# NVIDIA/flowtron

Measured on AMD Instinct MI355X. Metric: mel-frames/sec training (2-flow, 80-mel), higher is better.
Workload: dtype bf16; 1 GPU; BASELINE configs[1]: 2-flow LJS config.json model, per-GPU batch 32, T_max=862, L_max=157, attn-prior + CTC on, fwd+loss+bwd+clip+RAdam; global_batch=32, parallelism=dp1, mfma_operands=bf16, storage=fp32, skipped_steps=0

## Files before the change

### flowtron_amd/_lib.py

```python
from __future__ import annotations

import ctypes as C
import os

import torch

_HERE = os.path.dirname(os.path.abspath(__file__))
LIB_PATH = os.path.join(_HERE, "libflowtron_hip.so")

FT_F32, FT_BF16, FT_F16 = 0, 1, 2
GEMM_SPLITK = 1
GEMM_SPLITK_DET = 2
GEMM_C16 = 4
ACT_NONE, ACT_TANH, ACT_RELU, ACT_SIGMOID = 0, 1, 2, 3

_p, _i, _l, _f, _sz, _d = C.c_void_p, C.c_int, C.c_int64, C.c_float, C.c_size_t, C.c_double


class GemmArgs(C.Structure):
    _fields_ = [("A", _p), ("B", _p), ("C", _p), ("bias", _p),
                ("M", _i), ("N", _i), ("K", _i), ("batch", _i),
                ("sAm", _l), ("sAk", _l), ("sBk", _l), ("sBn", _l), ("ldc", _l),
                ("bsA", _l), ("bsB", _l), ("bsC", _l),
                ("alpha", _f), ("beta", _f), ("act", _i), ("mode", _i), ("flags", _i),
                ("work", _p), ("work_bytes", _sz)]


class GemmImgArgs(C.Structure):
    _fields_ = [("A", _p), ("B", _p), ("C", _p), ("bias", _p), ("M", _i), ("N", _i), ("K", _i),
                ("lda", _l), ("ldb", _l), ("ldc", _l), ("a_kmajor", _i), ("b_kmajor", _i),
                ("alpha", _f), ("beta", _f), ("act", _i), ("flags", _i),
                ("rowmap", _p), ("rows_dev", _p), ("compact", _i), ("k_shift", _i), ("r1_row", _p), ("r1_col", _p),
                ("split_work", _p), ("split_work_bytes", _sz)]


class LstmFwdRole(C.Structure):
    _fields_ = [("gx", _p), ("lens", _p), ("y", _p), ("ldy", _l), ("gates", _p), ("cell", _p), ("wimg", _p), ("state_h", _p), ("state_c", _p),
                ("B", C.c_int32), ("ldb", C.c_int32), ("t0", C.c_int32), ("t1", C.c_int32), ("gx16", C.c_int32)]


class LstmBwdRole(C.Structure):
    _fields_ = [("dy", _p), ("ldy", _l), ("lens", _p), ("gates", _p), ("cell", _p), ("dgx", _p), ("wimg", _p),
                ("dimg", _p), ("dimg_ld", _l), ("dimg_rows", _l), ("dbias", _p), ("state_da", _p), ("state_dc", _p),
                ("B", C.c_int32), ("ldb", C.c_int32), ("t0", C.c_int32), ("t1", C.c_int32), ("carry_in", C.c_int32)]


class ImgDesc(C.Structure):
    _fields_ = [("src", _p), ("ld", _l), ("rows", _l), ("cols", _l), ("dst", _p), ("kind", _i)]


class CummAttnArgs(C.Structure):
    _fields_ = [(n, _p) for n in ("text", "Q", "V", "w_key", "v", "w1", "b1", "w2", "b2", "in_lens", "ctx", "attn", "logprob",
                                  "cumm_all", "kproj_all", "work")] + [("work_bytes", _sz)] + [
        (n, _i) for n in ("T", "B", "L", "E", "A", "NF", "K1", "K2")] + [("temperature", _f), ("mode", _i), ("persist_status", _p)]


# ... 212 lines not shown
```

### flowtron_amd/csrc/gemm_bf16.hip

```cpp
#include "common.h"
#include <stdlib.h>

namespace {

constexpr int TB = 128;

inline size_t up(size_t v, size_t m) { return (v + m - 1) / m * m; }

__device__ __forceinline__ uint4 pack8(const float (&v)[8]) {
    uint4 o;
    o.x = pack_op16x2(v[0], v[1]); o.y = pack_op16x2(v[2], v[3]);
    o.z = pack_op16x2(v[4], v[5]); o.w = pack_op16x2(v[6], v[7]);
    return o;
}

__device__ __forceinline__ int mapped_rows(const int* rdev, int Rp, int& Rz) {
    const int R = *rdev;
    const int z = (R + 32 + 255) & ~255;
    Rz = z < Rp ? z : Rp;
    return R;
}

__device__ __forceinline__ void img_rows_body(const float* __restrict__ src, long sr, long sc, int R, int Cc,
                                              unsigned short* __restrict__ dst, int Rp, int Cp, int vec,
// ... 173 lines not shown
}

void make_image(const float* src, long sr, long sc, int R, int Cc, unsigned short* dst, int Rp, int Cp, hipStream_t st,
                const int* rowmap = nullptr, const int* rdev = nullptr, long dld = 0) {
    const bool vec = sc == 1 && reinterpret_cast<uintptr_t>(src) % 16 == 0 && sr % 4 == 0;
    const size_t chunks = (size_t)Rp * (Cp >> 3);
    const int blocks = (int)((chunks + 255) / 256 < 16384 ? (chunks + 255) / 256 : 16384);
    hipLaunchKernelGGL(img_rows_k, dim3(blocks), dim3(256), 0, st, src, sr, sc, R, Cc, dst, Rp, Cp, vec ? 1 : 0, rowmap, rdev,
                       dld ? dld : (long)Cp);
}

struct BfP {
    const unsigned short* A; const unsigned short* B; float* C; const float* bias;
    int M, N, nk;
    long lda, ldb, ldc;
    float alpha, beta;
    int act, gx, gy, splits, ksteps;
    int vec_c;
    const int* rowmap; const int* rows_dev; int compact, k_shift;
    int chunk_w;
    const float* r1row; const float* r1col;
    long c_slice;
    int c16;
};

typedef __attribute__((address_space(3))) void lds_void;
typedef const __attribute__((address_space(1))) void glb_void;
typedef __attribute__((ext_vector_type(4))) short bf16x4;

template <bool KM, int RT = 128>
struct Operand {
    static constexpr int NS = RT / 64;
    static constexpr int WT = RT / 32;
    const unsigned short* src[NS];
    size_t kstride;
    int dst[NS];
    int roff;
    __device__ __forceinline__ void init(const unsigned short* img, long ld, int r0, int wave, int lane, int wsel) {
        const int li = lane & 15, kg = lane >> 4;
        if constexpr (!KM) {
            const int srow = lane >> 2, skp = (lane & 3) ^ ((lane >> 4) & 2);
#pragma unroll
            for (int g = 0; g < NS; ++g) {
                src[g] = img + (size_t)(r0 + (wave * NS + g) * 16 + srow) * ld + skp * 8;
                dst[g] = (wave * NS + g) << 10;
            }
// ... 69 lines not shown
        for (int g = 0; g < NS; ++g)
            __builtin_amdgcn_global_load_lds((glb_void*)(src0 + (size_t)t * 64 + (size_t)g * ld8 + ((g & 1) ? xodd : 0)),
                                             (lds_void*)(sbuf + dst0 + g * 1024), 16, 0, 0);
    }
    __device__ __forceinline__ bf16x8 frag(const unsigned char* sbuf, int i, int ks) const {
        return *reinterpret_cast<const bf16x8*>(sbuf + ((roff + (i << 11)) ^ (ks << 6)));
    }
};

template <bool AKM, bool BKM, bool SPLIT, int RTA, int KS = 32, bool SB = false>
__global__ __launch_bounds__(256, SB ? 4 : (RTA == 256 || KS == 64) ? 2 : 4) void gemm_bf16_k(BfP p) {
    static_assert(!SB || (KS == 64 && RTA == 128 && !SPLIT), "single-buffer form: 128 x 128 x 64 store kernels");
    constexpr int KQ = KS / 32;
    constexpr int OPA = RTA * 64 * KQ, OPB = 8192 * KQ;
    constexpr int TI = RTA / 32;
    __shared__ __attribute__((aligned(1024))) unsigned char smem[(SB ? 1 : 2) * (OPA + OPB)];
    const int tid = threadIdx.x, lane = tid & 63, wave = tid >> 6;
    const int wm = wave >> 1, wn = wave & 1;
    const int li = lane & 15, kg = lane >> 4;
    int tile = blockIdx.x;
    int t0 = blockIdx.y * p.ksteps;
    int t1 = (t0 + p.ksteps < p.nk) ? t0 + p.ksteps : p.nk;
    int rows_lim = p.M, gy = p.gy;
    if (p.compact) {
        const int R = __builtin_amdgcn_readfirstlane(*p.rows_dev);
        if (p.compact == 1) {
            rows_lim = R < p.M ? R : p.M;
            gy = (rows_lim + RTA - 1) / RTA;
            if (gy == 0) return;
        } else {
            int nk_eff = (R - p.k_shift + 31) >> 5;
            nk_eff = nk_eff < p.nk ? nk_eff : p.nk;
            if constexpr (SPLIT) {
                const int ks = (nk_eff + (int)gridDim.y - 1) / (int)gridDim.y;
                t0 = blockIdx.y * ks;
                t1 = t0 + ks < nk_eff ? t0 + ks : nk_eff;
                if (t0 >= t1) return;
            } else t1 = t1 < nk_eff ? t1 : nk_eff;
        }
    }
    int mt, nt;
    if (p.chunk_w > 0 && gy >= 16) {
        const int xcd = tile & 7, idx = tile >> 3;
        const int qm = gy >> 3, rm = gy & 7;
        const int mh = qm + (xcd < rm ? 1 : 0);
        const int m_lo = xcd * qm + (xcd < rm ? xcd : rm);
        if (idx >= mh * p.gx) return;
        const int per_chunk = mh * p.chunk_w;
        const int ch = idx / per_chunk, within = idx - ch * per_chunk;
        const int left = p.gx - ch * p.chunk_w;
        const int cw = left < p.chunk_w ? left : p.chunk_w;
        const int mi = within / cw;
        mt = m_lo + mi;
        nt = ch * p.chunk_w + (within - mi * cw);
    } else {
        const int total = p.gx * gy, q = total >> 3, r = total & 7;
        const int xcd = tile & 7, idx = tile >> 3;
        if (tile >= total) return;
        tile = xcd * q + (xcd < r ? xcd : r) + idx;
        mt = tile / p.gx;
        nt = tile % p.gx;
    }
    const int m0 = mt * RTA, n0 = nt * TB;

    Operand<AKM, RTA> oa;
    Operand<BKM, 128> ob;
    Operand64<RTA> oa64;
    Operand64<128> ob64;
    if constexpr (KS == 64 && !AKM) oa64.init(p.A, p.lda, m0, wave, lane, wm); else oa.init(p.A, p.lda, m0, wave, lane, wm);
    if constexpr (KS == 64 && !BKM) ob64.init(p.B, p.ldb, n0, wave, lane, wn); else ob.init(p.B, p.ldb, n0, wave, lane, wn);

    f32x4 acc[TI][4];
#pragma unroll
    for (int i = 0; i < TI; ++i)
#pragma unroll
        for (int j = 0; j < 4; ++j) acc[i][j] = (f32x4){0.f, 0.f, 0.f, 0.f};

    auto issue_stage = [&](unsigned char* sbuf, int s) {
        if constexpr (KS == 64) {
            if constexpr (!AKM) oa64.issue(sbuf, s); else { oa.issue(sbuf, 2 * s); oa.issue(sbuf + OPA / 2, 2 * s + 1); }
            if constexpr (!BKM) ob64.issue(sbuf + OPA, s); else { ob.issue(sbuf + OPA, 2 * s); ob.issue(sbuf + OPA + OPB / 2, 2 * s + 1); }
        } else { oa.issue(sbuf, s); ob.issue(sbuf + OPA, s); }
    };
    auto load_frags = [&](const unsigned char* sbase, int ks, bf16x8 (&a)[TI], bf16x8 (&b)[4]) {
        const unsigned char* sa = sbase + ((KS == 64 && AKM) ? ks * (OPA / 2) : 0);
        const unsigned char* sb = sbase + OPA + ((KS == 64 && BKM) ? ks * (OPB / 2) : 0);
// ... 61 lines not shown
                load_frags(smem + stage * (OPA + OPB), ks, a, b);
                multiply(a, b);
            }
        }
    }

    if constexpr (SPLIT) {
#pragma unroll
        for (int i = 0; i < TI; ++i)
#pragma unroll
            for (int r = 0; r < 4; ++r) {
                int row = m0 + wm * (RTA / 2) + i * 16 + kg * 4 + r;
                if (row >= rows_lim) continue;
                if (p.compact == 1) { row = p.rowmap[row]; if (row < 0) continue; }
#pragma unroll
                for (int j = 0; j < 4; ++j) {
                    const int col = n0 + wn * 64 + j * 16 + li;
                    if (col >= p.N) continue;
                    float v = p.alpha * acc[i][j][r];
                    if (p.bias && blockIdx.y == 0) v += p.bias[col];
                    atomicAdd(p.C + (long)row * p.ldc + col, v);
                }
            }
        return;
    }

    const bool vec = p.vec_c != 0;
#pragma unroll
    for (int i = 0; i < TI; ++i) {
        int row = m0 + wm * (RTA / 2) + i * 16 + li;
        if (row >= rows_lim) continue;
        if (p.compact == 1) { row = p.rowmap[row]; if (row < 0) continue; }
#pragma unroll
        for (int j = 0; j < 4; ++j) {
            const int col = n0 + wn * 64 + j * 16 + kg * 4;
            if (col >= p.N) continue;
            float* cp = p.C + (size_t)blockIdx.y * p.c_slice + (long)row * p.ldc + col;
            float v[4] = {p.alpha * acc[i][j][0], p.alpha * acc[i][j][1], p.alpha * acc[i][j][2], p.alpha * acc[i][j][3]};
            const int nv = (p.N - col < 4) ? p.N - col : 4;
            const bool full = vec && nv == 4;
            if (p.beta != 0.f) {
                if (full) { const float4 c = *reinterpret_cast<const float4*>(cp); v[0] += p.beta * c.x; v[1] += p.beta * c.y; v[2] += p.beta * c.z; v[3] += p.beta * c.w; }
                else for (int r = 0; r < nv; ++r) v[r] += p.beta * cp[r];
            }
            const float r1 = p.r1row ? p.r1row[row] : 0.f;
#pragma unroll
// ... 52 lines not shown
    const long tiles_big = (long)cdiv(M, 256) * cdiv(N, TB);
    bool big = M >= 512 && can_split && tiles_big * (K / 512) >= 384;
    if (force_tile == 128) big = false;
    if (force_tile == 256) big = M >= 256;
    const int RTA = big ? 256 : TB;
    const long slots = big ? 512 : 1024;
    const long tiles = (long)cdiv(N, TB) * cdiv(M, RTA);
    long s = 1;
    if (can_split && tiles < slots / 2) {
        s = slots / tiles;
        const long smax = K / 512;
        if (s > smax) s = smax;
        if (s > 64) s = 64;
        if (s < 1) s = 1;
    }
    if (compact == 1) s = 1;
    *big_out = big;
    return s;
}

int run_images(const unsigned short* A, long lda, int a_km, const unsigned short* B, long ldb, int b_km, float* C, long ldc,
               const float* bias, int M, int N, int K, float alpha, float beta, int act, int flags, hipStream_t st,
               const int* rowmap = nullptr, const int* rows_dev = nullptr, int compact = 0, int k_shift = 0,
               const float* r1row = nullptr, const float* r1col = nullptr, float* split_work = nullptr, size_t split_work_bytes = 0) {
    BfP p;
    p.A = A; p.B = B; p.C = C; p.bias = bias;
    p.M = M; p.N = N; p.nk = cdiv(K, 32); p.lda = lda; p.ldb = ldb; p.ldc = ldc;
    p.alpha = alpha; p.beta = beta; p.act = act;
    p.rowmap = rowmap; p.rows_dev = rows_dev; p.compact = compact; p.k_shift = k_shift;
    p.r1row = r1row; p.r1col = r1col;
    p.c_slice = 0;
    p.c16 = (flags & FT_GEMM_C16) ? 1 : 0;
    if (p.c16 && (beta != 0.f || (flags & (FT_GEMM_SPLITK | FT_GEMM_SPLITK_DET))))
        return ft_fail(FT_EINVAL, "ft_gemm_img: FT_GEMM_C16 takes beta == 0 and no split-K");
    const bool det = (flags & FT_GEMM_SPLITK_DET) && split_work && act == FT_ACT_NONE && beta == 0.f && compact == 0 && !r1row && K >= 2048 &&
                     N % 4 == 0 && ldc % 4 == 0 && reinterpret_cast<uintptr_t>(C) % 16 == 0 && reinterpret_cast<uintptr_t>(split_work) % 16 == 0;
    const bool can_split = det || ((flags & FT_GEMM_SPLITK) && act == FT_ACT_NONE && (beta == 0.f || beta == 1.f) && K >= 2048 && !r1row);
    bool big;
    long s = plan_slices(M, N, K, can_split, compact, &big);
    const int RTA = big ? 256 : TB;
    p.gx = cdiv(N, TB); p.gy = cdiv(M, RTA);
    p.vec_c = (reinterpret_cast<uintptr_t>(C) % 16 == 0 && ldc % 4 == 0) ? 1 : 0;
    if (det) {
        const long fit = (long)(split_work_bytes / ((size_t)M * N * sizeof(float)));
        if (s > fit) s = fit;
        if (s < 1) s = 1;
    }
    const char* wide_env = getenv("FT_GEMM_BF16_WIDE");
    const bool wide = (!wide_env || atoi(wide_env) != 0) && (p.nk & 1) == 0 && !(a_km && b_km) && !big;
    p.ksteps = cdiv(p.nk, s);
    if (wide && (p.ksteps & 1)) ++p.ksteps;
    p.splits = cdiv(p.nk, p.ksteps);
    const bool det_on = det && p.splits > 1;
    if (det_on) {
        p.C = split_work; p.ldc = N; p.c_slice = (long)M * N; p.bias = nullptr;
        p.vec_c = 1;
    } else if (p.splits > 1 && beta == 0.f) {
        FT_CHECK_HIP(hipMemset2DAsync(C, sizeof(float) * ldc, 0, sizeof(float) * N, M, st));
    }
    static const int order_on = [] { const char* e = getenv("FT_GEMM_BF16_ORDER"); return e ? atoi(e) : 1; }();
    p.chunk_w = 0;
    int gridx = p.gx * p.gy;
    if (order_on && p.splits == 1 && p.gy >= 16) {
        long cw = (2l << 20) / ((long)TB * (long)p.nk * 32 * 2);
// ... 217 lines not shown
extern "C" int FT_OPNAME(ft_bf16_image_colsum)(const float* src, int64_t ld, int64_t rows, int64_t cols, void* dst, float* colsum, void* stream) {
    return image_colsum_impl(src, ld, rows, cols, dst, colsum, true, stream);
}
extern "C" int FT_OPNAME(ft_bf16_image_colsum_acc)(const float* src, int64_t ld, int64_t rows, int64_t cols, void* dst, float* colsum, void* stream) {
    return image_colsum_impl(src, ld, rows, cols, dst, colsum, false, stream);
}

#if FT_OPFMT == 0
extern "C" size_t ft_gemm_img_split_work_bytes(int M, int N, int K) {
    if (M < 1 || N < 1 || K < 2048 || N % 4 != 0) return 0;
    bool big;
    const long s = plan_slices(M, N, K, true, 0, &big);
    return s > 1 ? (size_t)s * M * N * sizeof(float) : 0;
}
#endif

extern "C" int FT_OPNAME(ft_gemm_img)(const ft_gemm_img_args* a, void* stream) {
    FT_CHECK_ARG(a != nullptr);
    FT_CHECK_ARG(a->A && a->B && a->C && a->M >= 1 && a->N >= 1 && a->K >= 1);
    FT_CHECK_ARG(a->lda % 8 == 0 && a->ldb % 8 == 0 && reinterpret_cast<uintptr_t>(a->A) % 16 == 0 && reinterpret_cast<uintptr_t>(a->B) % 16 == 0);
    FT_CHECK_ARG(a->compact >= 0 && a->compact <= 2 && (a->compact == 0 || a->rows_dev) && (a->compact != 1 || a->rowmap));
    FT_CHECK_ARG(a->k_shift >= 0 && (a->compact == 2 || a->k_shift == 0));
    FT_CHECK_ARG((a->r1_row == nullptr) == (a->r1_col == nullptr));
    return run_images(reinterpret_cast<const unsigned short*>(a->A), a->lda, a->a_kmajor, reinterpret_cast<const unsigned short*>(a->B),
                      a->ldb, a->b_kmajor, a->C, a->ldc, a->bias, a->M, a->N, a->K, a->alpha, a->beta, a->act, a->flags,
                      reinterpret_cast<hipStream_t>(stream), a->rowmap, a->rows_dev, a->compact, a->k_shift, a->r1_row, a->r1_col,
                      reinterpret_cast<float*>(a->split_work), a->split_work_bytes);
}

static int image_rows_act_bwd_impl(const float* dy, int64_t ld, const float* y, int64_t ldy, int act, int64_t cap_rows,
                                   int64_t cols, void* dst, float* colsum, const int32_t* rowmap,
                                   const int32_t* rows_dev, bool clear, void* stream) {
    FT_CHECK_ARG(dy && y && dst && colsum && rowmap && rows_dev && cap_rows >= 1 && cols >= 1 && ld >= cols && ldy >= cols);
    FT_CHECK_ARG(act >= FT_ACT_NONE && act <= FT_ACT_SIGMOID && cap_rows < (1ll << 31) - 512 && cols < (1ll << 31) - 256);
    FT_CHECK_ARG(reinterpret_cast<uintptr_t>(dst) % 256 == 0);
    hipStream_t st = reinterpret_cast<hipStream_t>(stream);
    const int Rp = (int)up((size_t)cap_rows + 32, 256), Cp = (int)up((size_t)cols, 256);
    const int vec = (reinterpret_cast<uintptr_t>(dy) % 16 == 0 && ld % 4 == 0 && reinterpret_cast<uintptr_t>(y) % 16 == 0 && ldy % 4 == 0) ? 1 : 0;
    if (clear) FT_CHECK_HIP(hipMemsetAsync(colsum, 0, sizeof(float) * (size_t)cols, st));
    hipLaunchKernelGGL(img_rows_sum_k, dim3(cdiv(Cp, 256), cdiv(Rp, IMG_SUM_SLAB)), dim3(256), 0, st, dy, (long)ld, (int)cap_rows, (int)cols,
                       reinterpret_cast<unsigned short*>(dst), Rp, Cp, vec, colsum, rowmap, rows_dev, y, (long)ldy, act);
    FT_CHECK_LAUNCH();
    return FT_OK;
}
extern "C" int FT_OPNAME(ft_bf16_image_rows_act_bwd)(const float* dy, int64_t ld, const float* y, int64_t ldy, int act, int64_t cap_rows,
                                                     int64_t cols, void* dst, float* colsum, const int32_t* rowmap,
                                                     const int32_t* rows_dev, void* stream) {
    return image_rows_act_bwd_impl(dy, ld, y, ldy, act, cap_rows, cols, dst, colsum, rowmap, rows_dev, true, stream);
}
extern "C" int FT_OPNAME(ft_bf16_image_rows_act_bwd_acc)(const float* dy, int64_t ld, const float* y, int64_t ldy, int act, int64_t cap_rows,
// ... 65 lines not shown
```

### flowtron_amd/model.py

```python
from __future__ import annotations

import ctypes as C
import numbers
import os
from typing import List, Optional

import torch
from torch import nn

from . import _lib as L
from . import ops



class LinearNorm(nn.Module):
    def __init__(self, in_dim, out_dim, bias=True, w_init_gain="linear"):
        super().__init__()
        self.linear_layer = nn.Linear(in_dim, out_dim, bias=bias)
        nn.init.xavier_uniform_(self.linear_layer.weight, gain=nn.init.calculate_gain(w_init_gain))

    def forward(self, x, act=L.ACT_NONE, rowmap=None, fill="y+dx"):
        return ops.linear(x, self.linear_layer.weight, self.linear_layer.bias, act, rowmap=rowmap, fill=fill)


# ... 8 lines not shown
        self.conv = nn.Conv1d(in_channels, out_channels, kernel_size=kernel_size, stride=stride,
                              padding=padding, dilation=dilation, bias=bias)
        nn.init.xavier_uniform_(self.conv.weight, gain=nn.init.calculate_gain(w_init_gain))


class MaskedInstanceNorm1d(nn.Module):

    def __init__(self, num_features, eps=1e-5, affine=True, **_):
        super().__init__()
        self.eps = eps
        self.weight = nn.Parameter(torch.ones(num_features))
        self.bias = nn.Parameter(torch.zeros(num_features))


class DenseLayer(nn.Module):
    def __init__(self, in_dim=1024, sizes=(1024, 1024)):
        super().__init__()
        sizes = list(sizes)
        in_sizes = [in_dim] + sizes[:-1]
        self.layers = nn.ModuleList([LinearNorm(i, o, bias=True) for i, o in zip(in_sizes, sizes)])

    def forward(self, x, rowmap=None):
        for lin in self.layers:
            x = lin(x, L.ACT_TANH, rowmap=rowmap, fill="")
        return x


class Encoder(nn.Module):
    def __init__(self, encoder_n_convolutions=3, encoder_embedding_dim=512, encoder_kernel_size=5,
                 norm_fn=MaskedInstanceNorm1d):
        super().__init__()
        convs = []
        for _ in range(encoder_n_convolutions):
            convs.append(nn.Sequential(
                ConvNorm(encoder_embedding_dim, encoder_embedding_dim, kernel_size=encoder_kernel_size, stride=1,
                         padding=int((encoder_kernel_size - 1) / 2), dilation=1, w_init_gain="relu"),
                norm_fn(encoder_embedding_dim, affine=True)))
        self.convolutions = nn.ModuleList(convs)
        self.lstm = nn.LSTM(encoder_embedding_dim, int(encoder_embedding_dim / 2), 1, batch_first=True,
                            bidirectional=True)
        self.dropout_masks = None

    def _run(self, x, lens):
        enc32 = os.environ.get("FLOWTRON_ENCODER_F32", "")
        conv_mode = L.FT_F32 if enc32 in ("conv", "all") else None
        lstm_mode = L.FT_F32 if enc32 == "all" else None
        m16 = L.mfma_mode()
# ... 86 lines not shown
        if add_gate:
            self.gate_threshold = 0.5
            self.gate_layer = LinearNorm(n_hidden + n_attn_channels, 1, bias=True, w_init_gain="sigmoid")
        self._decode_work = None

    def __getstate__(self):
        d = self.__dict__.copy()
        for k in ("_decode_bufs", "_decode_wimg", "_decode_gran", "_decode_batch_bufs", "_decode_batch_gran"):
            d.pop(k, None)
        d["_decode_work"] = None
        return d

    def forward(self, mel, text, in_lens32, out_lens32, attn_prior=None, rowmap=None):
        T, B, M = mel.shape
        mode = L.mfma_mode()
        rm = rowmap
        mel0 = torch.cat([mel.new_zeros(1, B, M), mel[:-1]], 0)
        a = self.attention_lstm
        h_att = ops.lstm_layer(mel0, out_lens32, a.weight_ih_l0, a.weight_hh_l0, a.bias_ih_l0, a.bias_hh_l0, mode=mode, rowmap=rm,
                               fill="dx")
        if self.use_cumm_attention:
            ctx, attn, logprob = self.run_cumm_attn_sequence(h_att, text, in_lens32)
        else:
            ctx, attn, logprob = self.attention_layer(h_att, text, text, in_lens32, attn_prior, rowmap=rm)
        gates = None
        p = self.lstm
        g = self.gate_layer.linear_layer if hasattr(self, "gate_layer") else None
        persist = (ops.lstm_persist_groups(B, p.weight_hh_l0.shape[1], False, mode, mel.device)
                   or bool(ops.lstm_persist_slices(B, p.weight_hh_l0.shape[1], False, mode, mel.device))
                   or ops.lstm_pad_width(B, p.weight_hh_l0.shape[1], False, mode, mel.device, T))
        fuse_gate = g is not None and (self.n_lstm_layers != 2 or persist or not ops.lstm2_supported(B, p.weight_hh_l0.shape[1], mode))
        if g is not None and not fuse_gate:
            gates = ops.linear([h_att, ctx], g.weight, g.bias, mode=mode)

        def first_layer():
            r = ops.lstm_layer(h_att, out_lens32, p.weight_ih_l0, p.weight_hh_l0, p.bias_ih_l0, p.bias_hh_l0, mode=mode,
                               xs_extra=[ctx], rowmap=rm, fill="dx", gate=(g.weight, g.bias) if fuse_gate else None)
            return r if fuse_gate else (r, gates)
        if self.n_lstm_layers != 2:
            h, gates = first_layer()
            for l in range(1, self.n_lstm_layers):
                h = ops.lstm_layer(h, out_lens32, getattr(p, "weight_ih_l%d" % l), getattr(p, "weight_hh_l%d" % l),
                                   getattr(p, "bias_ih_l%d" % l), getattr(p, "bias_hh_l%d" % l), mode=mode, rowmap=rm)
        elif persist and rm is not None and ops.decoder_pair_chunks(B, p.weight_hh_l0.shape[1], mode, mel.device, T):
            h, gates_f = ops.decoder_pair(h_att, out_lens32, p, mode, [ctx], rm, "dx", (g.weight, g.bias) if fuse_gate else None,
                                          ops.decoder_pair_chunks(B, p.weight_hh_l0.shape[1], mode, mel.device, T))
# ... 540 lines not shown
```

### flowtron_amd/ops.py

```python
from __future__ import annotations

import ctypes as C
from typing import List, Optional, Sequence

import torch

from . import _lib as L



def _c(t: torch.Tensor) -> torch.Tensor:
    return t if t.is_contiguous() else t.contiguous()


import os as _os
_BF16_IMAGES = True


def gemm_raw(A, B, Cm, M, N, K, sAm, sAk, sBk, sBn, ldc, bias=None, act=L.ACT_NONE, alpha=1.0, beta=0.0,
             batch=1, bsA=0, bsB=0, bsC=0, mode=None, splitk=False):
    L.require_cuda(A, B, Cm, bias)
    a = L.GemmArgs(L.ptr(A), L.ptr(B), L.ptr(Cm), L.ptr(bias), M, N, K, batch,
                   sAm, sAk, sBk, sBn, ldc, bsA, bsB, bsC, alpha, beta, act,
                   L.mfma_mode() if mode is None else mode, L.GEMM_SPLITK if splitk else 0,
# ... 104 lines not shown
            w["plan_next"][key] = W
        if w["armed"]:
            w["armed"] = False
            plan = [(k, t) for k, t in w["plan"].items() if t.is_cuda and t.device == W.device and t.dtype == torch.float32 and t.is_contiguous()
                    and t.data_ptr() == k[0] and tuple(t.shape) == k[1]]
            for lo in range(0, len(plan), 32):
                part = plan[lo:lo + 32]
                by_fmt = {}
                for k, t in part:
                    by_fmt.setdefault(k[2], []).append((k, t))
                for fmt, items in by_fmt.items():
                    descs = (L.ImgDesc * len(items))()
                    for i, (k, t) in enumerate(items):
                        img = cls._blank(t.shape[0], (3 if k[3] else 1) * t.shape[1], fmt, t.device)
                        descs[i] = L.ImgDesc(t.data_ptr(), int(t.stride(0)), int(t.shape[0]), int(t.shape[1]), img.buf.data_ptr(), 1 if k[3] else 0)
                        w["cache"][k] = img
                    L.check(L.op16("ft_bf16_image_table", fmt)(descs, len(items), L.stream()), "ft_bf16_image_table")
        img = w["cache"].get(key)
        if img is not None:
            return img
        return cls.split3(W, mode, True) if split else cls(W, mode=mode)

    @classmethod
    def cat_rows(cls, xs2d, mode, rowmap):
        self = cls.__new__(cls)
        self.rows, self.cols, self.fmt, self.rowmap, self.colsum = rowmap.cap, int(sum(x.shape[1] for x in xs2d)), mode, rowmap, None
        self.ld = (self.cols + 255) // 256 * 256
        self.buf = torch.empty(L.lib().ft_bf16_image_bytes(self.rows, self.cols), device=xs2d[0].device, dtype=torch.uint8)
        off = 0
        for i, x in enumerate(xs2d):
            assert x.dim() == 2 and x.stride(1) == 1 and x.dtype == torch.float32 and x.shape[0] == rowmap.T * rowmap.B
            K = int(x.shape[1])
            last = i == len(xs2d) - 1
            assert last or K % 8 == 0
            L.check(L.op16("ft_bf16_image_rows_into", mode)(L.ptr(x), int(x.stride(0)), self.rows, K, L.ptr(self.buf), self.ld, off,
                                                            (self.ld - off) if last else K, L.ptr(rowmap.map), L.ptr(rowmap.rows), L.stream()),
                    "ft_bf16_image_rows_into")
            off += K
        return self

    @classmethod
    def empty_rows(cls, cols, rowmap, mode, device):
        self = cls.__new__(cls)
        self.rows, self.cols, self.fmt, self.rowmap = rowmap.cap, int(cols), mode, rowmap
        self.ld = (self.cols + 255) // 256 * 256
        self.buf = torch.empty(L.lib().ft_bf16_image_bytes(self.rows, self.cols), device=device, dtype=torch.uint8)
        self.colsum = zeroed((self.cols,), device)
        return self


_WIMG_ON = True
_WIMG = {"plan": {}, "plan_next": None, "cache": {}, "armed": False, "plans": None}


def weight_images_begin(model):
    if not _WIMG_ON:
        return
# ... 14 lines not shown
import weakref as _weakref
_IMG_CACHE = {}


def shared_image(t, rows, cols, mode, rowmap=None):
    key = id(t)
    hit = _IMG_CACHE.get(key)
    want_rows = rows if rowmap is None else rowmap.cap
    if hit is not None:
        ref, ver, img = hit
        if ref() is t and ver == t._version and img.rows == want_rows and img.cols == cols and img.fmt == mode and img.rowmap is rowmap:
            return img
    img = Bf16Image(t.reshape(rows, cols), mode=mode, rowmap=rowmap)
    if len(_IMG_CACHE) > 64:
        for k in [k for k, (r, _, _) in _IMG_CACHE.items() if r() is None]:
            del _IMG_CACHE[k]
    try:
        _IMG_CACHE[key] = (_weakref.ref(t, lambda _r, k=key: _IMG_CACHE.pop(k, None)), t._version, img)
    except TypeError:
        pass
    return img


def op16_dtype(mode):
    return torch.float16 if mode == L.FT_F16 else torch.bfloat16


_GX16 = True


def gx16_ok(mode, rowmap, T, B, H, reverse, xs, N, device):
    return (_GX16 and L.is16(mode) and rowmap is not None and not reverse and rowmap.T == T and rowmap.B == B and _PERSIST_IMG == "1"
            and linear_uses_images(mode, T * B, N, xs) and (len(xs) == 1 or _CAT_IMAGES)
            and bool(lstm_persist_groups(B, H, reverse, mode, device) or lstm_persist_slices(B, H, reverse, mode, device))
            and B <= 32)


def images_apply(mode, M, N, K):
    return _BF16_IMAGES and L.is16(mode) and M >= 32 and N >= 32 and K >= 16 and M * N * K >= (1 << 20)


def gemm_img(A, a_km, a_ptr, B, b_km, b_ptr, Cm, M, N, K, ldc, bias=None, act=L.ACT_NONE, alpha=1.0, beta=0.0, splitk=False,
             rowmap=None, compact=0, k_shift=0, rank1=None, c16=False):
    L.require_cuda(Cm, bias)
    flags, work, need = (L.GEMM_SPLITK if splitk else 0), None, 0
    if splitk == "det":
        need = L.lib().ft_gemm_img_split_work_bytes(M, N, K)
        flags = L.GEMM_SPLITK_DET if need else 0
        work = torch.empty(need, device=Cm.device, dtype=torch.uint8) if need else None
    if c16:
        assert Cm.dtype == op16_dtype(A.fmt) and not splitk and beta == 0.0
        flags |= L.GEMM_C16
    a = L.GemmImgArgs(a_ptr, b_ptr, L.ptr(Cm), L.ptr(bias), M, N, K, A.ld, B.ld, ldc, int(a_km), int(b_km),
                      alpha, beta, act, flags,
                      L.ptr(rowmap.map) if rowmap is not None else None, L.ptr(rowmap.rows) if rowmap is not None else None,
                      int(compact) if rowmap is not None else 0, int(k_shift),
                      L.ptr(rank1[0]) if rank1 is not None else None, rank1[1] if rank1 is not None else None,
                      L.ptr(work), need)
    assert A.fmt == B.fmt, "operand images of different formats"
    L.check(L.op16("ft_gemm_img", A.fmt)(C.byref(a), L.stream()), "ft_gemm_img")


_HANDOFF = {"imgs": {}, "armed": False, "unwritten": set(), "nan_next": 0}
_NAN_POOL = {}


def _current_graph_task():
    try:
        return torch._C._current_graph_task_id()
    except Exception:
        return -1


def _handoff_clear():
    _HANDOFF["imgs"].clear()
    _HANDOFF["unwritten"].clear()
    _HANDOFF["armed"] = False
    _HANDOFF["nan_next"] = 0


def image_only_gradient(shape, device, dtype=torch.float32):
# ... 175 lines not shown
            assert len(xs) == 1 and act == L.ACT_NONE and L.is16(mode_dx) and mode_dx == mode_dw
            x2d = xs[0].reshape(rows, Ktot)
            split_imgs = lazy = None
            if Ktot % 32 == 0 and images_apply(mode_dx, rows, N, Ktot):
                lazy = _LAZY_COLS.pop(xs[0].data_ptr(), None)
                xi = Bf16Image.split3_im2col(*lazy, mode_dx) if lazy is not None else Bf16Image.split3(x2d, mode_dx, False)
                wi = Bf16Image.of_weight(W, mode_dx, split=True)
                gemm_img(xi, 0, xi.ptr(), wi, 0, wi.ptr(), y, rows, N, 3 * Ktot, N, bias=bias, splitk=_ENC_SPLITK)
                split_imgs = (wi.view_cols(Ktot), [xi.view_cols(Ktot)])
            else:
                _materialize_col(xs[0])
                gemm_raw(x2d, W, y, rows, N, Ktot, Ktot, 1, 1, Ktot, N, bias=bias, mode=L.FT_F32)
            mode = L.FT_F32
        mixed = not (mode == mode_dx == mode_dw)
        ctx.mode_dx, ctx.mode_dw = mode_dx, mode_dw
        use_img = (not mixed) and linear_uses_images(mode, rows, N, xs)
        ctx.lazy_img_mode = mode_dx if (mixed and mode_dx == mode_dw and linear_uses_images(mode_dx, rows, N, xs)) else None
        if rowmap is not None and (not use_img or rows != rowmap.T * rowmap.B):
            rowmap = None
        ctx.imgs = split_imgs if split_fwd else None
        ctx.cat = False
        ctx.img_kind = ("split3" if split_imgs is not None else None) if split_fwd else ("images" if use_img else None)
        ctx.lazy_src = lazy if split_fwd else None
        if use_img:
            w_img = Bf16Image.of_weight(W, mode)
            if len(xs) > 1 and rowmap is not None and _CAT_IMAGES:
                x_cat = Bf16Image.cat_rows([x.reshape(rows, x.shape[-1]) for x in xs], mode, rowmap)
                ctx.imgs, ctx.cat = (w_img, [x_cat]), True
                gemm_img(x_cat, 0, x_cat.ptr(), w_img, 0, w_img.ptr(), y, rowmap.cap, N, Ktot, N, bias=bias, act=act, rowmap=rowmap, compact=1, c16=c16)
            else:
                x_imgs = [shared_image(x, rows, x.shape[-1], mode, rowmap) for x in xs]
                ctx.imgs = (w_img, x_imgs)
        off = 0
        for i, x in enumerate(xs):
            if ctx.cat or split_fwd:
                off = Ktot
                break
            K = x.shape[-1]
            last = i == len(xs) - 1
            if use_img:
                assert not c16 or len(xs) == 1
                gemm_img(x_imgs[i], 0, x_imgs[i].ptr(), w_img, 0, w_img.ptr(0, off), y, rows if rowmap is None else rowmap.cap, N, K, N,
                         bias=bias if last else None, act=act if last else L.ACT_NONE, beta=0.0 if i == 0 else 1.0,
                         rowmap=rowmap, compact=1, c16=c16)
            else:
                assert not c16, "16-bit output rows come from the image GEMMs only"
                gemm_raw(x, W[:, off:], y, rows, N, K, K, 1, 1, Ktot, N,
                         bias=bias if last else None, act=act if last else L.ACT_NONE,
                         beta=0.0 if i == 0 else 1.0, mode=mode)
            off += K
        assert off == Ktot
        if rowmap is not None and "y" in fill:
            rowmap.fill(y.reshape(rows, N), N, copy_separator=True)
        ctx.save_for_backward(W, y if act != L.ACT_NONE else None, *xs)
        ctx.act, ctx.mode, ctx.has_bias, ctx.rowmap, ctx.fill = act, mode, bias is not None, rowmap, fill
        return y

    @staticmethod
    def backward(ctx, dy):
        W, y, *xs = ctx.saved_tensors
        N, Ktot = W.shape
        rows = dy.numel() // N
        rowmap = ctx.rowmap
        if ctx.imgs is None and ctx.img_kind is not None:
            ctx.imgs = _linear_images_again(ctx, W, xs, rows)
        elif ctx.imgs is None and ctx.lazy_img_mode is not None:
            lm = ctx.lazy_img_mode
            ctx.imgs = (Bf16Image(W, mode=lm), [shared_image(x, rows, x.shape[-1], lm, rowmap) for x in xs])
        d_img_in = _handoff_take(dy) if (ctx.act == L.ACT_NONE and ctx.imgs is not None) else None
        if d_img_in is not None and (d_img_in.fmt != ctx.imgs[0].fmt or d_img_in.rowmap is not rowmap
                                     or (ctx.has_bias and ctx.needs_input_grad[1] and d_img_in.colsum is None)):
            d_img_in = None
        if d_img_in is None:
            _require_written(dy)
            dy = _c(dy.float())
        fuse_act = ctx.act != L.ACT_NONE and ctx.imgs is not None and rowmap is not None and _FUSE_ACT_BWD
# ... 73 lines not shown


def linear_gate_fusable(mode, rowmap, xs, N):
    if not (_GATE_ON_CAT and _CAT_IMAGES and rowmap is not None and len(xs) == 2):
        return False
    rows = xs[0].numel() // xs[0].shape[-1]
    return rows == rowmap.T * rowmap.B and linear_uses_images(mode, rows, N, xs)


class LinearGateFn(torch.autograd.Function):

    @staticmethod
    def forward(ctx, W, bias, Wg, bg, mode, rowmap, fill, x0, x1):
        xs = [_c(x0), _c(x1)]
        L.require_cuda(W, Wg, *xs)
        W, Wg = _c(W), _c(Wg)
        N, Ktot = W.shape
        assert Wg.shape == (1, Ktot) and xs[0].shape[-1] + xs[1].shape[-1] == Ktot
        rows = rowmap.T * rowmap.B
        c16 = "c16" in fill
        y = torch.empty(xs[0].shape[:-1] + (N,), device=W.device, dtype=op16_dtype(mode) if c16 else torch.float32)
        gate = torch.empty(xs[0].shape[:-1] + (1,), device=W.device, dtype=torch.float32)
        w_img = Bf16Image.of_weight(W, mode)
        x_cat = Bf16Image.cat_rows([x.reshape(rows, x.shape[-1]) for x in xs], mode, rowmap)
        gemm_img(x_cat, 0, x_cat.ptr(), w_img, 0, w_img.ptr(), y, rowmap.cap, N, Ktot, N, bias=bias, rowmap=rowmap, compact=1, c16=c16)
        L.check(L.op16("ft_img_gemv_rows", mode)(L.ptr(x_cat.buf), x_cat.ld, Ktot, L.ptr(Wg), L.ptr(bg), L.ptr(gate), 1, L.ptr(rowmap.map),
                                                 L.ptr(rowmap.rows), L.ptr(rowmap.lens), rowmap.T, rowmap.B, L.stream()), "ft_img_gemv_rows")
        if "y" in fill:
            rowmap.fill(y.reshape(rows, N), N, copy_separator=True)
        ctx.save_for_backward(W, Wg, *xs)
        ctx.imgs = (w_img, x_cat)
        ctx.mode, ctx.has_bias, ctx.has_gbias, ctx.rowmap, ctx.fill = mode, bias is not None, bg is not None, rowmap, fill
        return y, gate

    @staticmethod
    def backward(ctx, dy, dgate):
        W, Wg, *xs = ctx.saved_tensors
        N, Ktot = W.shape
        rowmap = ctx.rowmap
        rows = rowmap.T * rowmap.B
        if ctx.imgs is None:
            ctx.imgs = (Bf16Image.of_weight(W, ctx.mode), Bf16Image.cat_rows([x.reshape(rows, x.shape[-1]) for x in xs], ctx.mode, rowmap))
        w_img, x_cat = ctx.imgs
        want_db = ctx.has_bias and ctx.needs_input_grad[1]
        d_img = _handoff_take(dy)
        if d_img is not None and (d_img.fmt != w_img.fmt or d_img.rowmap is not rowmap or (want_db and d_img.colsum is None)):
            d_img = None
# ... 1329 lines not shown
```

### include/flowtron_hip.h

```cpp
#ifndef FLOWTRON_HIP_H
#define FLOWTRON_HIP_H

#include <stddef.h>
#include <stdint.h>

#ifdef __cplusplus
extern "C" {
#endif

#define FT_ABI_VERSION 14

enum { FT_OK = 0, FT_EINVAL = -1, FT_EHIP = -2, FT_EUNSUPPORTED = -3 };
enum { FT_F32 = 0, FT_BF16 = 1, FT_F16 = 2 };
enum { FT_ACT_NONE = 0, FT_ACT_TANH = 1, FT_ACT_RELU = 2, FT_ACT_SIGMOID = 3 };
enum { FT_GEMM_SPLITK = 1, FT_GEMM_SPLITK_DET = 2, FT_GEMM_C16 = 4 };

int ft_abi_version(void);
const char* ft_last_error(void);
int ft_debug_hold_cus(int n_wg, int64_t ticks, void* stream);

typedef struct {
    const float* A; const float* B; float* C; const float* bias;
    int M, N, K, batch;
    int64_t sAm, sAk, sBk, sBn, ldc;
    int64_t bsA, bsB, bsC;
    float alpha, beta;
    int act, mode;
    int flags;
    void* work;
    size_t work_bytes;
} ft_gemm_args;
size_t ft_gemm_workspace_bytes(const ft_gemm_args* a);
int ft_gemm(const ft_gemm_args* a, void* stream);

typedef struct {
    const void* A; const void* B; float* C; const float* bias;
    int M, N, K;
    int64_t lda, ldb, ldc;
    int a_kmajor, b_kmajor;
    float alpha, beta;
    int act, flags;
    const int32_t* rowmap; const int32_t* rows_dev;
    int compact, k_shift;
    const float* r1_row; const float* r1_col;
    void* split_work; size_t split_work_bytes;
} ft_gemm_img_args;
size_t ft_gemm_img_split_work_bytes(int M, int N, int K);
size_t ft_bf16_image_bytes(int64_t rows, int64_t cols);
int ft_bf16_image(const float* src, int64_t ld, int64_t rows, int64_t cols, void* dst, void* stream);
int ft_bf16_image_colsum(const float* src, int64_t ld, int64_t rows, int64_t cols, void* dst, float* colsum, void* stream);
int ft_gemm_img(const ft_gemm_img_args* a, void* stream);
int ft_bf16_image_colsum_acc(const float* src, int64_t ld, int64_t rows, int64_t cols, void* dst, float* colsum, void* stream);
int ft_bf16_image_rows_acc(const float* src, int64_t ld, int64_t cap_rows, int64_t cols, void* dst, float* colsum,
                           const int32_t* rowmap, const int32_t* rows_dev, void* stream);
int ft_bf16_image_rows_act_bwd_acc(const float* dy, int64_t ld, const float* y, int64_t ldy, int act, int64_t cap_rows, int64_t cols,
                                   void* dst, float* colsum, const int32_t* rowmap, const int32_t* rows_dev, void* stream);
int ft_bf16_image_colsum_acc_f16(const float* src, int64_t ld, int64_t rows, int64_t cols, void* dst, float* colsum, void* stream);
int ft_bf16_image_rows_acc_f16(const float* src, int64_t ld, int64_t cap_rows, int64_t cols, void* dst, float* colsum,
                               const int32_t* rowmap, const int32_t* rows_dev, void* stream);
int ft_bf16_image_rows_act_bwd_acc_f16(const float* dy, int64_t ld, const float* y, int64_t ldy, int act, int64_t cap_rows, int64_t cols,
                                       void* dst, float* colsum, const int32_t* rowmap, const int32_t* rows_dev, void* stream);
int ft_bf16_image_split3(const float* src, int64_t ld, int64_t rows, int64_t cols, void* dst, int weight, void* stream);
int ft_bf16_image_split3_f16(const float* src, int64_t ld, int64_t rows, int64_t cols, void* dst, int weight, void* stream);
int ft_bf16_image_split3_im2col(const float* x, const int32_t* lens, int L, int B, int C, int KW, void* dst, void* stream);
int ft_bf16_image_split3_im2col_f16(const float* x, const int32_t* lens, int L, int B, int C, int KW, void* dst, void* stream);
typedef struct { const float* src; int64_t ld; int64_t rows; int64_t cols; void* dst; int kind; } ft_img_desc;
int ft_bf16_image_table(const ft_img_desc* descs, int n, void* stream);
int ft_bf16_image_table_f16(const ft_img_desc* descs, int n, void* stream);
// ... 298 lines not shown
```

Before: 689,800 mel-frames/s.

## Emit bf16 operand image from GEMM epilogue and pre-begin concat images

Adds an FT_GEMM_C_IMG mode in which the image GEMM epilogue also writes a packed 16-bit operand image of its output (zero-padded rows and columns) next to the fp32 C. The image is cached so later consumers skip a separate fp32-to-bf16 conversion pass. The prenet layers and the attention query input now start their concat image early, so cat_rows reuses the first block instead of converting it again. The cost is a larger epilogue with lane shuffles and extra stores, extra tiles launched to cover padding, and id/version-keyed cache bookkeeping on the Python side.

```diff
diff --git a/flowtron_amd/_lib.py b/flowtron_amd/_lib.py
--- a/flowtron_amd/_lib.py
+++ b/flowtron_amd/_lib.py
@@ -12,6 +12,7 @@
 GEMM_SPLITK = 1
 GEMM_SPLITK_DET = 2
 GEMM_C16 = 4
+GEMM_C_IMG = 8
 ACT_NONE, ACT_TANH, ACT_RELU, ACT_SIGMOID = 0, 1, 2, 3
 
 _p, _i, _l, _f, _sz, _d = C.c_void_p, C.c_int, C.c_int64, C.c_float, C.c_size_t, C.c_double
@@ -31,7 +32,8 @@
                 ("lda", _l), ("ldb", _l), ("ldc", _l), ("a_kmajor", _i), ("b_kmajor", _i),
                 ("alpha", _f), ("beta", _f), ("act", _i), ("flags", _i),
                 ("rowmap", _p), ("rows_dev", _p), ("compact", _i), ("k_shift", _i), ("r1_row", _p), ("r1_col", _p),
-                ("split_work", _p), ("split_work_bytes", _sz)]
+                ("split_work", _p), ("split_work_bytes", _sz),
+                ("img", _p), ("img_ld", _l), ("img_fill", _l)]
 
 
 class LstmFwdRole(C.Structure):
diff --git a/flowtron_amd/csrc/gemm_bf16.hip b/flowtron_amd/csrc/gemm_bf16.hip
--- a/flowtron_amd/csrc/gemm_bf16.hip
+++ b/flowtron_amd/csrc/gemm_bf16.hip
@@ -1,4 +1,5 @@
 #include "common.h"
+#include "gemm_img_epilogue.h"
 #include <stdlib.h>
 
 namespace {
@@ -219,6 +220,7 @@
     const float* r1row; const float* r1col;
     long c_slice;
     int c16;
+    unsigned short* img; long img_ld; int img_fill, img_rp;
 };
 
 typedef __attribute__((address_space(3))) void lds_void;
@@ -334,11 +336,16 @@
     int t0 = blockIdx.y * p.ksteps;
     int t1 = (t0 + p.ksteps < p.nk) ? t0 + p.ksteps : p.nk;
     int rows_lim = p.M, gy = p.gy;
+    int img_rz = p.img_rp;
     if (p.compact) {
         const int R = __builtin_amdgcn_readfirstlane(*p.rows_dev);
         if (p.compact == 1) {
             rows_lim = R < p.M ? R : p.M;
             gy = (rows_lim + RTA - 1) / RTA;
+            if (p.img) {
+                img_rz = ft_img_epi_rows(R, p.M);
+                gy = img_rz / RTA;
+            }
             if (gy == 0) return;
         } else {
             int nk_eff = (R - p.k_shift + 31) >> 5;
@@ -374,6 +381,7 @@
         nt = tile % p.gx;
     }
     const int m0 = mt * RTA, n0 = nt * TB;
+    if (p.img && (m0 >= rows_lim || n0 >= p.N)) t0 = t1 = 0;
 
     Operand<AKM, RTA> oa;
     Operand<BKM, 128> ob;
@@ -481,6 +489,52 @@
                     atomicAdd(p.C + (long)row * p.ldc + col, v);
                 }
             }
+        return;
+    }
+
+    if (p.img) {
+        const ft_img_epi_geo geo = {RTA, img_rz, p.img_fill, p.img_ld};
+        const bool vec = p.vec_c != 0;
+        const bool odd = (kg & 1) != 0;
+#pragma unroll
+        for (int i = 0; i < TI; ++i) {
+            const int irow = m0 + wm * (RTA / 2) + i * 16 + li;
+            int row = irow;
+            bool live = irow < rows_lim;
+            if (live && p.compact == 1) { row = p.rowmap[irow]; live = row >= 0; }
+            const float r1 = (live && p.r1row) ? p.r1row[row] : 0.f;
+            unsigned int pk[4][2];
+#pragma unroll
+            for (int j = 0; j < 4; ++j) {
+                const int col = n0 + wn * 64 + j * 16 + kg * 4;
+                const int nv = p.N - col < 0 ? 0 : (p.N - col < 4 ? p.N - col : 4);
+                float v[4] = {p.alpha * acc[i][j][0], p.alpha * acc[i][j][1], p.alpha * acc[i][j][2], p.alpha * acc[i][j][3]};
+#pragma unroll
+                for (int r = 0; r < 4; ++r) {
+                    if (r < nv && p.bias) v[r] += p.bias[col + r];
+                    if (r < nv && p.r1row) v[r] = fmaf(r1, p.r1col[col + r], v[r]);
+                    if (p.act == FT_ACT_TANH) v[r] = tanhf_(v[r]);
+                    else if (p.act == FT_ACT_RELU) v[r] = fmaxf(v[r], 0.f);
+                    else if (p.act == FT_ACT_SIGMOID) v[r] = sigmoidf_(v[r]);
+                    if (!live || r >= nv) v[r] = 0.f;
+                }
+                if (live && nv > 0) {
+                    float* cp = p.C + (long)row * p.ldc + col;
+                    if (vec && nv == 4) *reinterpret_cast<float4*>(cp) = make_float4(v[0], v[1], v[2], v[3]);
+                    else for (int r = 0; r < nv; ++r) cp[r] = v[r];
+                }
+                pk[j][0] = pack_op16x2(v[0], v[1]);
+                pk[j][1] = pack_op16x2(v[2], v[3]);
+            }
+#pragma unroll
+            for (int jp = 0; jp < 2; ++jp) {
+                const unsigned int s0_ = odd ? pk[2 * jp][0] : pk[2 * jp + 1][0], s1_ = odd ? pk[2 * jp][1] : pk[2 * jp + 1][1];
+                const unsigned int g0 = (unsigned int)__shfl_xor((int)s0_, 16), g1 = (unsigned int)__shfl_xor((int)s1_, 16);
+                const uint4 out = odd ? make_uint4(g0, g1, pk[2 * jp + 1][0], pk[2 * jp + 1][1]) : make_uint4(pk[2 * jp][0], pk[2 * jp][1], g0, g1);
+                const long o = ft_img_epi_offset(geo, m0, n0, wm, wn, lane, i, jp);
+                if (o >= 0) *reinterpret_cast<uint4*>(p.img + o) = out;
+            }
+        }
         return;
     }
 
@@ -579,7 +633,8 @@
 int run_images(const unsigned short* A, long lda, int a_km, const unsigned short* B, long ldb, int b_km, float* C, long ldc,
                const float* bias, int M, int N, int K, float alpha, float beta, int act, int flags, hipStream_t st,
                const int* rowmap = nullptr, const int* rows_dev = nullptr, int compact = 0, int k_shift = 0,
-               const float* r1row = nullptr, const float* r1col = nullptr, float* split_work = nullptr, size_t split_work_bytes = 0) {
+               const float* r1row = nullptr, const float* r1col = nullptr, float* split_work = nullptr, size_t split_work_bytes = 0,
+               unsigned short* img = nullptr, long img_ld = 0, int img_fill = 0) {
     BfP p;
     p.A = A; p.B = B; p.C = C; p.bias = bias;
     p.M = M; p.N = N; p.nk = cdiv(K, 32); p.lda = lda; p.ldb = ldb; p.ldc = ldc;
@@ -590,6 +645,9 @@
     p.c16 = (flags & FT_GEMM_C16) ? 1 : 0;
     if (p.c16 && (beta != 0.f || (flags & (FT_GEMM_SPLITK | FT_GEMM_SPLITK_DET))))
         return ft_fail(FT_EINVAL, "ft_gemm_img: FT_GEMM_C16 takes beta == 0 and no split-K");
+    p.img = (flags & FT_GEMM_C_IMG) ? img : nullptr; p.img_ld = img_ld; p.img_fill = img_fill; p.img_rp = 0;
+    if ((flags & FT_GEMM_C_IMG) && (!img || beta != 0.f || compact == 2 || (flags & (FT_GEMM_SPLITK | FT_GEMM_SPLITK_DET | FT_GEMM_C16))))
+        return ft_fail(FT_EINVAL, "ft_gemm_img: FT_GEMM_C_IMG takes an image, beta == 0, no split-K, no 16-bit C and no compact reduction");
     const bool det = (flags & FT_GEMM_SPLITK_DET) && split_work && act == FT_ACT_NONE && beta == 0.f && compact == 0 && !r1row && K >= 2048 &&
                      N % 4 == 0 && ldc % 4 == 0 && reinterpret_cast<uintptr_t>(C) % 16 == 0 && reinterpret_cast<uintptr_t>(split_work) % 16 == 0;
     const bool can_split = det || ((flags & FT_GEMM_SPLITK) && act == FT_ACT_NONE && (beta == 0.f || beta == 1.f) && K >= 2048 && !r1row);
@@ -597,6 +655,11 @@
     long s = plan_slices(M, N, K, can_split, compact, &big);
     const int RTA = big ? 256 : TB;
     p.gx = cdiv(N, TB); p.gy = cdiv(M, RTA);
+    if (p.img) {
+        p.img_rp = (int)up((size_t)M + 32, 256);
+        p.gy = p.img_rp / RTA;
+        if (cdiv(img_fill, TB) > p.gx) p.gx = cdiv(img_fill, TB);
+    }
     p.vec_c = (reinterpret_cast<uintptr_t>(C) % 16 == 0 && ldc % 4 == 0) ? 1 : 0;
     if (det) {
         const long fit = (long)(split_work_bytes / ((size_t)M * N * sizeof(float)));
@@ -860,10 +923,17 @@
     FT_CHECK_ARG(a->compact >= 0 && a->compact <= 2 && (a->compact == 0 || a->rows_dev) && (a->compact != 1 || a->rowmap));
     FT_CHECK_ARG(a->k_shift >= 0 && (a->compact == 2 || a->k_shift == 0));
     FT_CHECK_ARG((a->r1_row == nullptr) == (a->r1_col == nullptr));
+    int img_fill = 0;
+    if (a->flags & FT_GEMM_C_IMG) {
+        img_fill = a->img_fill ? (int)a->img_fill : (a->N + 7) & ~7;
+        FT_CHECK_ARG(a->img && reinterpret_cast<uintptr_t>(a->img) % 16 == 0 && a->img_ld % 8 == 0 && a->img_fill >= 0 && a->img_fill % 8 == 0);
+        FT_CHECK_ARG(img_fill >= a->N && img_fill <= a->img_ld && a->img_fill < (1ll << 31) - 256 && a->M < (1ll << 31) - 512);
+    }
     return run_images(reinterpret_cast<const unsigned short*>(a->A), a->lda, a->a_kmajor, reinterpret_cast<const unsigned short*>(a->B),
                       a->ldb, a->b_kmajor, a->C, a->ldc, a->bias, a->M, a->N, a->K, a->alpha, a->beta, a->act, a->flags,
                       reinterpret_cast<hipStream_t>(stream), a->rowmap, a->rows_dev, a->compact, a->k_shift, a->r1_row, a->r1_col,
-                      reinterpret_cast<float*>(a->split_work), a->split_work_bytes);
+                      reinterpret_cast<float*>(a->split_work), a->split_work_bytes, reinterpret_cast<unsigned short*>(a->img), (long)a->img_ld,
+                      img_fill);
 }
 
 static int image_rows_act_bwd_impl(const float* dy, int64_t ld, const float* y, int64_t ldy, int act, int64_t cap_rows,
diff --git a/flowtron_amd/csrc/gemm_img_epilogue.h b/flowtron_amd/csrc/gemm_img_epilogue.h
--- /dev/null
+++ b/flowtron_amd/csrc/gemm_img_epilogue.h
@@ -0,0 +1,33 @@
+#pragma once
+
+#if defined(__HIPCC__) || defined(__CUDACC__)
+#define FT_IMG_HD __host__ __device__ __forceinline__
+#else
+#define FT_IMG_HD inline
+#endif
+
+struct ft_img_epi_geo {
+    int rta;
+    int rz, fill;
+    long ld;
+};
+
+FT_IMG_HD int ft_img_epi_rows(int R, int cap) {
+    const int z = (R + 32 + 255) & ~255, rp = (cap + 32 + 255) & ~255;
+    return z < rp ? z : rp;
+}
+
+FT_IMG_HD int ft_img_epi_col(int n0, int wn, int lane, int jp) {
+    const int kg = lane >> 4;
+    return n0 + wn * 64 + (2 * jp + (kg & 1)) * 16 + (kg >> 1) * 8;
+}
+
+FT_IMG_HD int ft_img_epi_row(const ft_img_epi_geo& g, int m0, int wm, int lane, int i) {
+    return m0 + wm * (g.rta / 2) + i * 16 + (lane & 15);
+}
+
+FT_IMG_HD long ft_img_epi_offset(const ft_img_epi_geo& g, int m0, int n0, int wm, int wn, int lane, int i, int jp) {
+    const int row = ft_img_epi_row(g, m0, wm, lane, i), col = ft_img_epi_col(n0, wn, lane, jp);
+    if (row >= g.rz || col >= g.fill) return -1;
+    return (long)row * g.ld + col;
+}
diff --git a/flowtron_amd/model.py b/flowtron_amd/model.py
--- a/flowtron_amd/model.py
+++ b/flowtron_amd/model.py
@@ -54,7 +54,7 @@
 
     def forward(self, x, rowmap=None):
         for lin in self.layers:
-            x = lin(x, L.ACT_TANH, rowmap=rowmap, fill="")
+            x = lin(x, L.ACT_TANH, rowmap=rowmap, fill="img")
         return x
 
 
@@ -187,6 +187,8 @@
         if self.use_cumm_attention:
             ctx, attn, logprob = self.run_cumm_attn_sequence(h_att, text, in_lens32)
         else:
+            if rm is not None:
+                ops.cat_image_begin(h_att, self.attention_layer.value.linear_layer.weight.shape[0], mode, rm)
             ctx, attn, logprob = self.attention_layer(h_att, text, text, in_lens32, attn_prior, rowmap=rm)
         gates = None
         p = self.lstm
diff --git a/flowtron_amd/ops.py b/flowtron_amd/ops.py
--- a/flowtron_amd/ops.py
+++ b/flowtron_amd/ops.py
@@ -150,17 +150,22 @@
         return cls.split3(W, mode, True) if split else cls(W, mode=mode)
 
     @classmethod
-    def cat_rows(cls, xs2d, mode, rowmap):
-        self = cls.__new__(cls)
-        self.rows, self.cols, self.fmt, self.rowmap, self.colsum = rowmap.cap, int(sum(x.shape[1] for x in xs2d)), mode, rowmap, None
-        self.ld = (self.cols + 255) // 256 * 256
-        self.buf = torch.empty(L.lib().ft_bf16_image_bytes(self.rows, self.cols), device=xs2d[0].device, dtype=torch.uint8)
+    def cat_rows(cls, xs2d, mode, rowmap, first=None):
+        begun = _cat_image_take(first, int(sum(x.shape[1] for x in xs2d)), mode, rowmap) if first is not None else None
+        self = begun if begun is not None else cls.__new__(cls)
+        if begun is None:
+            self.rows, self.cols, self.fmt, self.rowmap, self.colsum = rowmap.cap, int(sum(x.shape[1] for x in xs2d)), mode, rowmap, None
+            self.ld = (self.cols + 255) // 256 * 256
+            self.buf = torch.empty(L.lib().ft_bf16_image_bytes(self.rows, self.cols), device=xs2d[0].device, dtype=torch.uint8)
         off = 0
         for i, x in enumerate(xs2d):
             assert x.dim() == 2 and x.stride(1) == 1 and x.dtype == torch.float32 and x.shape[0] == rowmap.T * rowmap.B
             K = int(x.shape[1])
             last = i == len(xs2d) - 1
             assert last or K % 8 == 0
+            if begun is not None and i == 0:
+                off += K
+                continue
             L.check(L.op16("ft_bf16_image_rows_into", mode)(L.ptr(x), int(x.stride(0)), self.rows, K, L.ptr(self.buf), self.ld, off,
                                                             (self.ld - off) if last else K, L.ptr(rowmap.map), L.ptr(rowmap.rows), L.stream()),
                     "ft_bf16_image_rows_into")
@@ -221,6 +226,41 @@
     return img
 
 
+_GEMM_C_IMG = True
+_CAT_PENDING = {}
+
+
+def _cache_image(t, img):
+    key = id(t)
+    try:
+        _IMG_CACHE[key] = (_weakref.ref(t, lambda _r, k=key: _IMG_CACHE.pop(k, None)), t._version, img)
+    except TypeError:
+        pass
+
+
+def cat_image_begin(x, extra_cols, mode, rowmap):
+    K = int(x.shape[-1])
+    if not (_GEMM_C_IMG and _CAT_IMAGES and _BF16_IMAGES and rowmap is not None and L.is16(mode) and x.is_cuda and x.dtype == torch.float32
+            and x.is_contiguous() and K % 64 == 0 and x.numel() // K == rowmap.T * rowmap.B):
+        return
+    img = Bf16Image._blank(rowmap.cap, K + int(extra_cols), mode, x.device)
+    img.rowmap = rowmap
+    L.check(L.op16("ft_bf16_image_rows_into", mode)(L.ptr(x), K, img.rows, K, L.ptr(img.buf), img.ld, 0, K, L.ptr(rowmap.map), L.ptr(rowmap.rows),
+                                                    L.stream()), "ft_bf16_image_rows_into")
+    _cache_image(x, img.view_cols(K))
+    key = id(x)
+    _CAT_PENDING[key] = (_weakref.ref(x, lambda _r, k=key: _CAT_PENDING.pop(k, None)), x._version, img)
+
+
+def _cat_image_take(x, cols, mode, rowmap):
+    hit = _CAT_PENDING.pop(id(x), None)
+    if hit is not None:
+        ref, ver, img = hit
+        if ref() is x and ver == x._version and img.cols == cols and img.fmt == mode and img.rowmap is rowmap:
+            return img
+    return None
+
+
 def op16_dtype(mode):
     return torch.float16 if mode == L.FT_F16 else torch.bfloat16
 
@@ -240,7 +280,7 @@
 
 
 def gemm_img(A, a_km, a_ptr, B, b_km, b_ptr, Cm, M, N, K, ldc, bias=None, act=L.ACT_NONE, alpha=1.0, beta=0.0, splitk=False,
-             rowmap=None, compact=0, k_shift=0, rank1=None, c16=False):
+             rowmap=None, compact=0, k_shift=0, rank1=None, c16=False, c_img=None):
     L.require_cuda(Cm, bias)
     flags, work, need = (L.GEMM_SPLITK if splitk else 0), None, 0
     if splitk == "det":
@@ -250,12 +290,16 @@
     if c16:
         assert Cm.dtype == op16_dtype(A.fmt) and not splitk and beta == 0.0
         flags |= L.GEMM_C16
+    if c_img is not None:
+        assert not splitk and beta == 0.0 and not c16 and c_img.fmt == A.fmt and c_img.rows == M and c_img.cols == N and compact != 2
+        flags |= L.GEMM_C_IMG
     a = L.GemmImgArgs(a_ptr, b_ptr, L.ptr(Cm), L.ptr(bias), M, N, K, A.ld, B.ld, ldc, int(a_km), int(b_km),
                       alpha, beta, act, flags,
                       L.ptr(rowmap.map) if rowmap is not None else None, L.ptr(rowmap.rows) if rowmap is not None else None,
                       int(compact) if rowmap is not None else 0, int(k_shift),
                       L.ptr(rank1[0]) if rank1 is not None else None, rank1[1] if rank1 is not None else None,
-                      L.ptr(work), need)
+                      L.ptr(work), need,
+                      c_img.ptr() if c_img is not None else None, c_img.ld if c_img is not None else 0, c_img.ld if c_img is not None else 0)
     assert A.fmt == B.fmt, "operand images of different formats"
     L.check(L.op16("ft_gemm_img", A.fmt)(C.byref(a), L.stream()), "ft_gemm_img")
 
@@ -477,12 +521,17 @@
         ctx.cat = False
         ctx.img_kind = ("split3" if split_imgs is not None else None) if split_fwd else ("images" if use_img else None)
         ctx.lazy_src = lazy if split_fwd else None
+        y_img = None
+        if "img" in fill and _GEMM_C_IMG and use_img and rowmap is not None and not c16 and (len(xs) == 1 or _CAT_IMAGES):
+            y_img = Bf16Image._blank(rowmap.cap, N, mode, W.device)
+            y_img.rowmap = rowmap
         if use_img:
             w_img = Bf16Image.of_weight(W, mode)
             if len(xs) > 1 and rowmap is not None and _CAT_IMAGES:
-                x_cat = Bf16Image.cat_rows([x.reshape(rows, x.shape[-1]) for x in xs], mode, rowmap)
+                x_cat = Bf16Image.cat_rows([x.reshape(rows, x.shape[-1]) for x in xs], mode, rowmap, first=xs[0])
                 ctx.imgs, ctx.cat = (w_img, [x_cat]), True
-                gemm_img(x_cat, 0, x_cat.ptr(), w_img, 0, w_img.ptr(), y, rowmap.cap, N, Ktot, N, bias=bias, act=act, rowmap=rowmap, compact=1, c16=c16)
+                gemm_img(x_cat, 0, x_cat.ptr(), w_img, 0, w_img.ptr(), y, rowmap.cap, N, Ktot, N, bias=bias, act=act, rowmap=rowmap, compact=1, c16=c16,
+                         c_img=y_img)
             else:
                 x_imgs = [shared_image(x, rows, x.shape[-1], mode, rowmap) for x in xs]
                 ctx.imgs = (w_img, x_imgs)
@@ -497,7 +546,7 @@
                 assert not c16 or len(xs) == 1
                 gemm_img(x_imgs[i], 0, x_imgs[i].ptr(), w_img, 0, w_img.ptr(0, off), y, rows if rowmap is None else rowmap.cap, N, K, N,
                          bias=bias if last else None, act=act if last else L.ACT_NONE, beta=0.0 if i == 0 else 1.0,
-                         rowmap=rowmap, compact=1, c16=c16)
+                         rowmap=rowmap, compact=1, c16=c16, c_img=y_img)
             else:
                 assert not c16, "16-bit output rows come from the image GEMMs only"
                 gemm_raw(x, W[:, off:], y, rows, N, K, K, 1, 1, Ktot, N,
@@ -507,6 +556,8 @@
         assert off == Ktot
         if rowmap is not None and "y" in fill:
             rowmap.fill(y.reshape(rows, N), N, copy_separator=True)
+        if y_img is not None:
+            _cache_image(y, y_img)
         ctx.save_for_backward(W, y if act != L.ACT_NONE else None, *xs)
         ctx.act, ctx.mode, ctx.has_bias, ctx.rowmap, ctx.fill = act, mode, bias is not None, rowmap, fill
         return y
@@ -626,7 +677,7 @@
         y = torch.empty(xs[0].shape[:-1] + (N,), device=W.device, dtype=op16_dtype(mode) if c16 else torch.float32)
         gate = torch.empty(xs[0].shape[:-1] + (1,), device=W.device, dtype=torch.float32)
         w_img = Bf16Image.of_weight(W, mode)
-        x_cat = Bf16Image.cat_rows([x.reshape(rows, x.shape[-1]) for x in xs], mode, rowmap)
+        x_cat = Bf16Image.cat_rows([x.reshape(rows, x.shape[-1]) for x in xs], mode, rowmap, first=xs[0])
         gemm_img(x_cat, 0, x_cat.ptr(), w_img, 0, w_img.ptr(), y, rowmap.cap, N, Ktot, N, bias=bias, rowmap=rowmap, compact=1, c16=c16)
         L.check(L.op16("ft_img_gemv_rows", mode)(L.ptr(x_cat.buf), x_cat.ld, Ktot, L.ptr(Wg), L.ptr(bg), L.ptr(gate), 1, L.ptr(rowmap.map),
                                                  L.ptr(rowmap.rows), L.ptr(rowmap.lens), rowmap.T, rowmap.B, L.stream()), "ft_img_gemv_rows")
diff --git a/include/flowtron_hip.h b/include/flowtron_hip.h
--- a/include/flowtron_hip.h
+++ b/include/flowtron_hip.h
@@ -13,7 +13,7 @@
 enum { FT_OK = 0, FT_EINVAL = -1, FT_EHIP = -2, FT_EUNSUPPORTED = -3 };
 enum { FT_F32 = 0, FT_BF16 = 1, FT_F16 = 2 };
 enum { FT_ACT_NONE = 0, FT_ACT_TANH = 1, FT_ACT_RELU = 2, FT_ACT_SIGMOID = 3 };
-enum { FT_GEMM_SPLITK = 1, FT_GEMM_SPLITK_DET = 2, FT_GEMM_C16 = 4 };
+enum { FT_GEMM_SPLITK = 1, FT_GEMM_SPLITK_DET = 2, FT_GEMM_C16 = 4, FT_GEMM_C_IMG = 8 };
 
 int ft_abi_version(void);
 const char* ft_last_error(void);
@@ -44,6 +44,7 @@
     int compact, k_shift;
     const float* r1_row; const float* r1_col;
     void* split_work; size_t split_work_bytes;
+    void* img; int64_t img_ld; int64_t img_fill;
 } ft_gemm_img_args;
 size_t ft_gemm_img_split_work_bytes(int M, int N, int K);
 size_t ft_bf16_image_bytes(int64_t rows, int64_t cols);
```

Result: no change. 689,300 mel-frames/s (-0.1%).
